# uzh-rpg/rpg_monocular_pose_estimator

Hardware: AMD Instinct MI355X
Metric: frames/sec at 752x480, 5 LEDs, brute-force init; pose RMSE vs CPU ref (higher is better)
Workload: dtype f64; 1 GPU; C2: 752x480 synthetic frames, 5 LEDs, 0 distractors, brute-force P3P init every frame, demo.launch parameters; frames_resident_in_hbm=True, side_streams_concurrent=1, scan_split_pct=28, side_scan_blocks=1, entry=mpe_estimate_batch_device_submit / _collect, parallelism=frames sharded over 1 GPU(s), pose records gathered to rank 0

## Files before the change

rpg_monocular_pose_estimator_amd/binding.py:

```python
import ctypes as C
import os
import re
import subprocess

import numpy as np

_HERE = os.path.dirname(os.path.abspath(__file__))
_CSRC = os.path.join(_HERE, "csrc")
_LIB = os.environ.get("MPE_LIB") or os.path.join(_HERE, "libmpe_hip.so")
_HEADER = os.path.join(os.path.dirname(_HERE), "include", "mpe.h")

MAX_MARKERS = 16
MAX_DETECTIONS = int(os.environ.get("MPE_MAX_DET", "64"))
WIDE_DETECTIONS = 256


class MpeError(RuntimeError):
    pass


class MpeParams(C.Structure):
    _fields_ = [
        ("threshold_value", C.c_int),
        ("gaussian_sigma", C.c_double),
        ("min_blob_area", C.c_double),
        ("max_blob_area", C.c_double),
        ("max_width_height_distortion", C.c_double),
        ("max_circular_distortion", C.c_double),
        ("back_projection_pixel_tolerance", C.c_double),
        ("nearest_neighbour_pixel_tolerance", C.c_double),
        ("certainty_threshold", C.c_double),
        ("valid_correspondence_threshold", C.c_double),
        ("roi_border_thickness", C.c_uint),
        ("histogram_threshold", C.c_uint),
    ]


class MpeResult(C.Structure):
    _fields_ = [("T", C.c_double * 16), ("cov", C.c_double * 36), ("status", C.c_int), ("n_det", C.c_int),
                ("n_corr", C.c_int), ("gn_iterations", C.c_int)]


class MpeDetections(C.Structure):
    _fields_ = [("n", C.c_int), ("status", C.c_int), ("undist_xy", C.c_double * (2 * MAX_DETECTIONS)),
                ("dist_xy", C.c_float * (2 * MAX_DETECTIONS))]


class MpeDetectionsWide(C.Structure):
    _fields_ = [("n", C.c_int), ("status", C.c_int), ("undist_xy", C.c_double * (2 * WIDE_DETECTIONS)),
                ("dist_xy", C.c_float * (2 * WIDE_DETECTIONS))]


RESULT_DTYPE = np.dtype([("T", "f8", (16,)), ("cov", "f8", (36,)), ("status", "i4"), ("n_det", "i4"),
                         ("n_corr", "i4"), ("gn_iterations", "i4")])
DETECTIONS_DTYPE = np.dtype([("n", "i4"), ("status", "i4"), ("undist_xy", "f8", (2 * MAX_DETECTIONS,)),
                             ("dist_xy", "f4", (2 * MAX_DETECTIONS,))])
assert RESULT_DTYPE.itemsize == C.sizeof(MpeResult)
DETECTIONS_WIDE_DTYPE = np.dtype([("n", "i4"), ("status", "i4"), ("undist_xy", "f8", (2 * WIDE_DETECTIONS,)),
                                  ("dist_xy", "f4", (2 * WIDE_DETECTIONS,))])
assert DETECTIONS_DTYPE.itemsize == C.sizeof(MpeDetections)
assert DETECTIONS_WIDE_DTYPE.itemsize == C.sizeof(MpeDetectionsWide)


def library_path():
    return _LIB


def build_library(force=False):
    cmd = ["make", "-s", "-j4", "-C", _CSRC] + (["-B"] if force else [])
    subprocess.check_call(cmd)
    if not os.path.exists(_LIB):
        raise MpeError("build did not produce %s" % _LIB)
    return _LIB


DEVICE_SOURCES = ("mpe_kernels_common.h", "mpe_k1.hip", "mpe_k2_head.h", "mpe_k2.hip", "mpe_k3.hip")


def device_source():
    out = []
    for name in DEVICE_SOURCES:
        with open(os.path.join(_CSRC, name)) as fh:
            txt = fh.read()
        txt = re.sub(r"//@file-prologue\n.*?//@file-prologue-end\n", "", txt, flags=re.S)
        txt = re.sub(r"//@file-epilogue\n.*?//@file-epilogue-end\n", "", txt, flags=re.S)
        if "//@include-k1b-dev" in txt:
            with open(os.path.join(_CSRC, "mpe_k1b_dev.h")) as fh:
                hdr = fh.read()
            body = hdr[hdr.index("//@k1b-dev-begin\n") + len("//@k1b-dev-begin\n"):hdr.index("//@k1b-dev-end\n")]
            txt = re.sub(r"//@include-k1b-dev.*?//@include-k1b-dev-end\n", lambda m: body, txt, count=1, flags=re.S)
        out.append(txt)
    return "".join(out)


def source_fingerprint():
    import hashlib
    hsh = hashlib.sha256()
    for name in DEVICE_SOURCES + ("mpe_k1b_dev.h", "mpe_ddmath.h", "mpe_p3p.h", "mpe_internal.h", "mpe_host.h", "mpe_schedule.cpp",
                                  "mpe_options.cpp", "mpe_track_abi.cpp", "mpe_abi.cpp", "mpe_track_device.hip",
                                  "mpe_gather.h", "mpe_pixel.h", "mpe_brute_blocks.h", "mpe_wide_peel.h", "mpe_wide.cpp"):
        with open(os.path.join(_CSRC, name), "rb") as fh:
            hsh.update(fh.read())
    return hsh.hexdigest()[:16]


def exported_symbols():
    txt = open(_HEADER).read()
    txt = re.sub(r"/\*.*?\*/", "", txt, flags=re.S)
    return sorted(set(re.findall(r"\b(mpe_[a-z0-9_]+)\s*\(", txt)))


_lib = None


def load_library():
    global _lib
    if _lib is not None:
        return _lib
    if not os.path.exists(_LIB):
        raise MpeError("%s is missing: run __graft_entry__.build() / make -C %s (there is no CPU fallback)"
                       % (_LIB, _CSRC))
    try:
        import torch
    except Exception:
        pass
    lib = C.CDLL(_LIB)
    lib.mpe_version.restype = C.c_char_p
    lib.mpe_last_error.restype = C.c_char_p
    lib.mpe_last_error.argtypes = [C.c_void_p]
    lib.mpe_get_stream.restype = C.c_void_p
    lib.mpe_get_stream.argtypes = [C.c_void_p]
    lib.mpe_create.argtypes = [C.POINTER(C.c_void_p), C.c_int]
    lib.mpe_destroy.argtypes = [C.c_void_p]
    lib.mpe_destroy.restype = None
    lib.mpe_set_stream.argtypes = [C.c_void_p, C.c_void_p]
    lib.mpe_synchronize.argtypes = [C.c_void_p]
    lib.mpe_set_profiling.argtypes = [C.c_void_p, C.c_int]
    lib.mpe_last_kernel_ms.argtypes = [C.c_void_p, C.POINTER(C.c_float)]
    lib.mpe_last_launch_shape.argtypes = [C.c_void_p, C.POINTER(C.c_int), C.POINTER(C.c_int)]
    lib.mpe_set_option.argtypes = [C.c_void_p, C.c_char_p, C.c_int]
    lib.mpe_default_params.argtypes = [C.POINTER(MpeParams)]
    lib.mpe_default_params.restype = None
    dp = C.POINTER(C.c_double)
    lib.mpe_find_leds.argtypes = [C.c_void_p, C.c_void_p, C.c_int, C.c_int, C.c_size_t, C.c_int, C.c_int, C.c_int,
                                  C.c_int, C.POINTER(MpeParams), dp, dp, C.c_int, dp, C.POINTER(C.c_float), C.c_int,
                                  C.POINTER(C.c_int)]
    lib.mpe_solve_bruteforce.argtypes = [C.c_void_p, dp, C.c_int, dp, C.c_int, dp, C.POINTER(MpeParams),
                                         C.POINTER(MpeResult), C.POINTER(C.c_uint32), C.POINTER(C.c_uint32)]
    ip, up = C.POINTER(C.c_int), C.POINTER(C.c_uint32)
    lib.mpe_solve_bruteforce_batch.argtypes = [C.c_void_p, dp, ip, C.c_int, dp, C.c_int, dp, C.POINTER(MpeParams),
                                               C.c_void_p, up, up]
    lib.mpe_solve_bruteforce_batch_setups.argtypes = [C.c_void_p, dp, ip, ip, C.c_int, C.c_void_p, C.c_int, C.c_void_p,
                                                      up, up]
    lib.mpe_estimate_batch.argtypes = [C.c_void_p, C.c_void_p, C.c_int, C.c_int, C.c_int, C.c_size_t, C.c_size_t,
                                       C.c_int, dp, C.c_int, dp, dp, C.c_int, C.POINTER(MpeParams), C.c_void_p]
    lib.mpe_estimate_batch_device.argtypes = [C.c_void_p, C.c_void_p, C.c_int, C.c_int, C.c_int, dp, C.c_int, dp, dp,
                                              C.c_int, C.POINTER(MpeParams), C.c_void_p]
    lib.mpe_estimate_batch_device_submit.argtypes = [C.c_void_p, C.c_void_p, C.c_int, C.c_int, C.c_int, dp, C.c_int, dp,
                                                     dp, C.c_int, C.POINTER(MpeParams), C.c_void_p, C.c_void_p, C.c_int]
    lib.mpe_estimate_batch_device_collect.argtypes = [C.c_void_p, C.c_void_p]
    lib.mpe_stream_next_ready.argtypes = [C.c_void_p, C.c_void_p]
    lib.mpe_stream_drop_prefetch.argtypes = [C.c_void_p]
    lib.mpe_track_step_batch_collect.argtypes = [C.c_void_p, C.c_void_p, C.c_void_p, C.c_void_p]
    lib.mpe_track_step_batch_cancel.argtypes = [C.c_void_p]
    lib.mpe_estimate_batch_multi_device_gather.argtypes = [C.c_void_p, C.c_int, C.c_void_p, C.c_void_p, C.c_int, C.c_int, dp,
                                                           C.c_int, dp, dp, C.c_int, C.POINTER(MpeParams), C.c_void_p,
                                                           C.POINTER(C.c_int)]
    lib.mpe_convert_to_mono8.argtypes = [C.c_void_p, C.c_void_p, C.c_int, C.c_int, C.c_int, C.c_int, C.c_int, C.c_int,
                                         C.c_size_t, C.c_size_t, C.c_void_p, C.c_int]
    lib.mpe_detect_batch.argtypes = [C.c_void_p, C.c_void_p, C.c_int, C.c_int, C.c_int, C.c_size_t, C.c_size_t, C.c_int,
                                     dp, dp, C.c_int, C.POINTER(MpeParams), C.c_void_p]
    lib.mpe_vote_batch.argtypes = [C.c_void_p, dp, C.POINTER(C.c_int), C.c_int, dp, C.c_int, dp, C.c_double,
                                   C.POINTER(C.c_uint32)]
    lib.mpe_vote_batch_wide.argtypes = lib.mpe_vote_batch.argtypes
    lib.mpe_detect_batch_wide.argtypes = lib.mpe_detect_batch.argtypes
    lib.mpe_estimate_batch_wide.argtypes = lib.mpe_estimate_batch.argtypes
    lib.mpe_solve_bruteforce_batch_wide.argtypes = lib.mpe_solve_bruteforce_batch.argtypes
    lib.mpe_vote_items.argtypes = [C.c_void_p, dp, C.POINTER(C.c_int), C.c_int, dp, C.c_int, dp, C.c_double,
                                   C.POINTER(C.c_int), C.POINTER(C.c_int), C.POINTER(C.c_uint32)]
    lib.mpe_check_and_refine.argtypes = [C.c_void_p, dp, C.c_int, dp, C.c_int, dp, C.POINTER(MpeParams),
                                         C.POINTER(C.c_uint32), C.c_int, C.POINTER(MpeResult)]
    lib.mpe_tracker_create.argtypes = [C.c_void_p, C.POINTER(C.c_void_p)]
    lib.mpe_tracker_destroy.argtypes = [C.c_void_p]
# ... 830 lines not shown
```

rpg_monocular_pose_estimator_amd/csrc/mpe_internal.h:

```cpp
#pragma once
#include <hip/hip_runtime.h>
#include <stdint.h>

#include "../../include/mpe.h"
#include "mpe_brute_blocks.h"

namespace mpe {

struct FrameGeom {
  int rows, cols, pitch;
  int segs_per_row;
  int segs_per_frame;
  int wb;
  int rw;
  int tw;
  int slot_cap;
};

struct DetectParams {
  int thr;
  int ksize;
  int taps[MPE_MAX_KSIZE];
  double min_area, max_area, max_wh, max_circ;
  double K[9];
  double ifx, ify;
  double k[8];
  int undist_iters;
  int roi_x, roi_y;
  unsigned taps_packed[2];
  int taps_u8;
};
inline void pack_taps(DetectParams& dp) {
  dp.taps_packed[0] = dp.taps_packed[1] = 0;
  dp.taps_u8 = 1;
  for (int i = 0; i < dp.ksize && i < MPE_MAX_KSIZE; ++i) {
    if (dp.taps[i] < 0 || dp.taps[i] > 255) dp.taps_u8 = 0;
    if (i < 8) dp.taps_packed[i >> 2] |= ((unsigned)dp.taps[i] & 0xFFu) << (8 * (i & 3));
  }
}

struct SolveParams {
  int n_markers;
  double markers[MPE_MAX_MARKERS * 3];
  double fx, fy, cx, cy;
  double back_tol;
  double certainty_thr;
  double valid_corr_thr;
  unsigned hist_thr;
  int vote_arith;
  int refine_variant;
};

__host__ __device__ inline bool vote_arith_is_strict(int a) { return a == 0 || a == 4; }
__host__ __device__ inline bool vote_arith_screens(int a) { return a == 1 || a == 3; }
__host__ __device__ inline bool vote_arith_glibc_pow(int a) { return a == 3 || a == 4; }

#define MPE_HIST_WORDS (MPE_MAX_DETECTIONS * MPE_MAX_MARKERS)
#define MPE_HIST_STRIDE (MPE_HIST_WORDS + 32)
#define MPE_WIDE_HIST_WORDS (MPE_WIDE_DETECTIONS * MPE_MAX_MARKERS)
#define MPE_WIDE_HIST_STRIDE (MPE_WIDE_HIST_WORDS + 32)

#define MPE_FIX_CTL_WORDS 8
struct VoteFixup {
  unsigned* ctl;
  unsigned long long* list;
  unsigned cap;
  unsigned screen;
};

int device_cu_count();
size_t k1b_scratch_bytes(const FrameGeom& g, int n_frames);
void k1b_set_general_blocks(int cap);
int k1b_get_general_blocks();
hipError_t launch_k1a_scan(const uint8_t* frames, size_t n_bytes, unsigned long long* flags, int thr,
                           int dummy_lds_bytes, hipStream_t s, int blocks_per_cu = 0);
hipError_t launch_k1b_blobs(const uint8_t* frames, const unsigned long long* flags, int n_frames, const FrameGeom& g,
                            const DetectParams& dp, mpe_detections* dets, int* worklist, uint8_t* scratch,
                            size_t scratch_bytes, int blob_hint, hipStream_t s, const void* frame_windows = nullptr,
                            bool lists_zeroed = false, bool first_tier_only = false, bool general_lds = false);
size_t k2_table_bytes(int n_markers);
hipError_t launch_k2_prep(const SolveParams& sp, double* tab, hipStream_t s);
hipError_t launch_k2_vote(mpe_detections* dets, int n_frames, const SolveParams& sp, const double* tab,
                          uint32_t* hist, int splits, int n_det_hint, hipStream_t s, const uint8_t* scan_px = nullptr,
                          size_t scan_bytes = 0, unsigned long long* scan_flags = nullptr, int scan_thr = 0,
                          size_t* scanned_bytes = nullptr, const int* item_range = nullptr,
                          const VoteFixup* fixup = nullptr);
hipError_t launch_k2_fixup(mpe_detections* dets, int n_frames, const SolveParams& sp, uint32_t* hist,
                           const VoteFixup& fixup, hipStream_t s, int relost_blocks = 32,
                           const int* item_range = nullptr);
int k2_table_slices(int n_markers);
size_t k3_mid_bytes(int n_frames);
hipError_t launch_k3_tail(const mpe_detections* dets, const uint32_t* hist, int n_frames, const SolveParams& sp,
                          mpe_result* results, uint32_t* corr_out, const uint32_t* corr_in, const double* nn_pred,
                          double nn_tol, void* mid_buf, hipStream_t s, int mode = 0);
struct TrackFramesArgs {
  const uint8_t* pix;
  size_t slot_bytes;
  const double* pred;
  const void* wins;
// ... 46 lines not shown
```

rpg_monocular_pose_estimator_amd/csrc/mpe_k1b_dev.h:

```cpp
#pragma once
#include "mpe_kernels_common.h"
namespace mpe {
struct BlobRec {
  long long a00, a10, a01;
  int xmin, xmax, ymin, ymax;
};
#ifndef K1B_ON_BLOBREC
#define K1B_ON_BLOBREC(rec, key)
#endif

__device__ __forceinline__ int reflect101(int p, int len) {
  if ((unsigned)p < (unsigned)len) return p;
  if (len == 1) return 0;
  do {
    p = (p < 0) ? -p : 2 * (len - 1) - p;
  } while ((unsigned)p >= (unsigned)len);
  return p;
}

__device__ __forceinline__ void lds_set_range(u64* bits, int lo, int hi) {
  const int wl = lo >> 6, wh = hi >> 6;
  if (wl == wh) {
    const u64 m = (~0ull << (lo & 63)) & (~0ull >> (63 - (hi & 63)));
    atomicOr(&bits[wl], m);
// ... 905 lines not shown
    if (over) st = MPE_FRAME_TOO_MANY_ROWS;
    out->status = st;
  }
}

struct FrameWin {
  int rows, cols, roi_x, roi_y;
};
__device__ __forceinline__ FrameGeom window_geom(const FrameGeom& g, const FrameWin* wins, int f, const DetectParams& dp,
                                                 int& roi_x, int& roi_y) {
  FrameGeom gl = g;
  roi_x = dp.roi_x;
  roi_y = dp.roi_y;
  if (wins) {
    const FrameWin w = wins[f];
    gl.rows = w.rows;
    gl.cols = w.cols;
    roi_x = w.roi_x;
    roi_y = w.roi_y;
  }
  return gl;
}

struct Island {
  short ylo, yhi;
  short clo, chi;
  short cfirst, clast;
  int pix_off, bm_off;
  int stage_end, blur_end;
  short blo, bhi;
};

#ifdef K1B_WIDE_WINDOWS
__device__ __forceinline__ int isl_xw0(const Island& is, int) { return 16 * is.clo; }
__device__ __forceinline__ int isl_words(const Island& is, int cols, int) {
  return ((min(cols - 1, 16 * is.chi + 15) - 16 * is.clo + 1) + 2 + 63) / 64;
}
#else
__device__ __forceinline__ int isl_xw0(const Island& is, int r) { return max(16 * is.clo, 16 * is.cfirst - r); }
__device__ __forceinline__ int isl_words(const Island& is, int cols, int r) {
  const int xhi = min(min(cols - 1, 16 * is.chi + 15), 16 * is.clast + 15 + r);
  return ((xhi - isl_xw0(is, r) + 1) + 2 + 63) / 64;
}
#endif
#ifndef K1B_SMALL_WAVES
#define K1B_SMALL_WAVES 1
#endif
#ifndef K1B_SMALL_MIN_WAVES
#define K1B_SMALL_MIN_WAVES 4
#endif
#ifndef K1B_SMALL_PIX
#define K1B_SMALL_PIX 4096
#endif
#ifndef K1B_SMALL_BM
#define K1B_SMALL_BM 208
#endif
struct K1bSmall {
  enum { PIX = K1B_SMALL_PIX, BM = K1B_SMALL_BM, SEG = 64, BAND = 8, ISL = 8, KEPT = 16, WAVES = K1B_SMALL_WAVES, MIN_WAVES = K1B_SMALL_MIN_WAVES };
};
struct K1bLarge {
  enum { PIX = 12288, BM = 704, SEG = 512, BAND = 32, ISL = 32, KEPT = 64, WAVES = 1, MIN_WAVES = 2 };
};


template <class C>
struct K1bWaveLds {
  enum { SCRATCH = 4 * C::SEG + 512 + 32 * C::BAND + 4 * C::BAND, POOL = C::PIX > SCRATCH ? C::PIX : SCRATCH };
  __attribute__((aligned(16))) uint8_t pool[POOL];
  int taps[MPE_MAX_KSIZE];
  int nseg, nband;
  int blur_go;
#ifdef K1B_PHASE_CLOCKS
  unsigned long long clk[8];
#endif
};
#ifdef K1B_PHASE_CLOCKS
#define K1B_PHASE_STAMP(W, i) \
  if ((threadIdx.x & 63) == 0) (W).clk[i] = __builtin_amdgcn_s_memtime();
#else
#define K1B_PHASE_STAMP(W, i)
#endif
template <class C>
struct K1bFrameLds {
  u64 nz[C::BM + 1], pm[C::BM + 1], ng[C::BM + 1];
  Island isl[C::ISL];
  float kx[C::KEPT], ky[C::KEPT];
  unsigned kkey[C::KEPT];
  int nkept, over, nisl;
  int ready, cols, roi_x, roi_y;
};

#ifdef K1B_STOP_AFTER
#define K1B_STOP_POINT(PHASE, REC) \
  if (K1B_STOP_AFTER <= (PHASE)) { \
    if (lane == 0) {               \
      (REC)->n = 0;                \
      (REC)->status = 0;           \
    }                              \
    return false;                  \
  }
#else
#define K1B_STOP_POINT(PHASE, REC)
#endif
template <class C>
__device__ __forceinline__ void k1b_blur_items(K1bWaveLds<C>& W, K1bFrameLds<C>& S, const FrameGeom& g, const DetectParams& dp,
                                               int tid, int nthr) {
  const Island* s_isl = S.isl;
  const int nisl = S.nisl, r = dp.ksize / 2;
  const int tot_blur = s_isl[nisl - 1].blur_end;
  for (int i = tid; i < tot_blur; i += nthr) {
    int k = 0;
    while (i >= s_isl[k].blur_end) ++k;
    const Island is = s_isl[k];
    const int li = i - (k ? s_isl[k - 1].blur_end : 0);
    const int ncols = is.bhi - is.blo + 1;
    const int yb = li / ncols, c = is.blo + (li - yb * ncols);
    const int H = is.yhi - is.ylo + 1;
    const int Wd = isl_words(is, g.cols, r);
    const PixWin pw = {W.pool + is.pix_off, is.ylo, H, is.cfirst, 16 * (is.clast - is.cfirst + 1), 0u, nullptr, 0};
    blur_to_bitmap(pw, g.rows, g.cols, dp, W.taps, is.ylo + yb, c, S.nz + is.bm_off + (size_t)(yb + 1) * Wd, isl_xw0(is, r));
  }
}

template <class C, bool HELP = false>
__device__ __forceinline__ bool k1b_front(const int f, const uint8_t* __restrict__ frames, size_t slot_bytes,
                                          const u64* __restrict__ flags, const FrameGeom& g, const DetectParams& dp,
                                          mpe_detections* __restrict__ dets, int* __restrict__ worklist,
                                          K1bWaveLds<C>& W, K1bFrameLds<C>& S) {
  const int lane = threadIdx.x & 63;
  unsigned* s_seg = reinterpret_cast<unsigned*>(W.pool);
  u64* s_rowact = reinterpret_cast<u64*>(W.pool + 4 * C::SEG);
  u64(*s_colocc)[4] = reinterpret_cast<u64(*)[4]>(W.pool + 4 * C::SEG + 512);
  short* s_bandlo = reinterpret_cast<short*>(W.pool + 4 * C::SEG + 512 + 32 * C::BAND);
  short* s_bandhi = s_bandlo + C::BAND;
  uint8_t* s_pix = W.pool;
  int& s_nseg = W.nseg;
  int& s_nband = W.nband;
  u64 *s_nz = S.nz, *s_pm = S.pm, *s_ng = S.ng;
  Island* s_isl = S.isl;
  int& s_nkept = S.nkept;
  int& s_over = S.over;
  int& s_nisl = S.nisl;
  const uint8_t* frame = frames + (size_t)f * slot_bytes;
  mpe_detections* out = dets + f;
  const int r = dp.ksize / 2;
  const int dc = (r + 15) / 16;
  const int spr = g.segs_per_row;
  const unsigned add = (unsigned)(255 - dp.thr) * 0x00010001u;

  s_rowact[lane] = 0;
  for (int i = lane; i < C::BAND * 4; i += 64) (&s_colocc[0][0])[i] = 0;
  if (lane == 0) {
    s_nseg = 0;
    s_nkept = 0;
    s_over = 0;
    s_nband = 0;
    s_nisl = 0;
  }
  wave_sync();

  {
    const size_t G0 = (size_t)f * g.segs_per_frame;
    const int nwin = (g.segs_per_frame + 63) >> 6;
    const size_t w0 = G0 >> 6;
    const int sh = (int)(G0 & 63);
    for (int i0 = 0; i0 < nwin; i0 += 256) {
      u64 v[4];
#pragma unroll
      for (int k = 0; k < 4; ++k) {
        const int i = i0 + 64 * k + lane;
        v[k] = 0;
        if (i < nwin) {
          const u64 a = flags[w0 + i], b = flags[w0 + i + 1];
          v[k] = sh ? ((a >> sh) | (b << (64 - sh))) : a;
          const int rem = g.segs_per_frame - i * 64;
          if (rem < 64) v[k] &= (1ull << rem) - 1;
        }
      }
#pragma unroll
      for (int k = 0; k < 4; ++k) {
        u64 vv = v[k];
        const int i = i0 + 64 * k + lane;
        while (vv) {
          const int s = i * 64 + __builtin_ctzll(vv);
          vv &= vv - 1;
          const int y0 = s / spr, c0 = s - y0 * spr;
          const int slot = atomicAdd(&s_nseg, 1);
          if (slot < C::SEG) s_seg[slot] = ((unsigned)y0 << 16) | (unsigned)c0;
          lds_set_range(s_rowact, max(0, y0 - r), min(g.rows - 1, y0 + r));
        }
      }
    }
  }
  wave_sync();
  const int nseg = s_nseg;
  if (nseg == 0) {
    if (lane == 0) {
      out->n = 0;
      out->status = 0;
    }
    return false;
  }
  K1B_STOP_POINT(1, out)
  K1B_PHASE_STAMP(W, 1)
  bool fallback = nseg > C::SEG;
  int why = fallback ? 1 : 0;

  {
    const u64 act = (lane < g.rw) ? s_rowact[lane] : 0;
    const u64 prevw = (lane > 0 && lane < g.rw) ? s_rowact[lane - 1] : 0;
    const u64 nextw = (lane + 1 < g.rw) ? s_rowact[lane + 1] : 0;
    u64 st = act & ~((act << 1) | (prevw >> 63));
    u64 en = act & ~((act >> 1) | (nextw << 63));
    const int cs = __builtin_popcountll(st), ce = __builtin_popcountll(en);
    int ps = cs, pe = ce;
#pragma unroll
    for (int d = 1; d < 64; d <<= 1) {
      const int a = __shfl_up(ps, d), b = __shfl_up(pe, d);
      if (lane >= d) {
        ps += a;
        pe += b;
      }
    }
    int is_ = ps - cs, ie = pe - ce;
    if (!fallback) {
      while (st) {
        const int b = __builtin_ctzll(st);
        st &= st - 1;
        if (is_ < C::BAND) s_bandlo[is_] = (short)(lane * 64 + b);
        ++is_;
      }
      while (en) {
        const int b = __builtin_ctzll(en);
        en &= en - 1;
        if (ie < C::BAND) s_bandhi[ie] = (short)(lane * 64 + b);
        ++ie;
      }
    }
    if (lane == 63) s_nband = ps;
  }
  wave_sync();
  const int nband = s_nband;
  fallback = fallback || nband > C::BAND;
  if (fallback && !why) why = 2;

  if (!fallback) {
    for (int i = lane; i < nseg; i += 64) {
      const unsigned sg = s_seg[i];
      const int y = (int)(sg >> 16), c = (int)(sg & 0xFFFF);
      int b = 0;
      while (b < nband - 1 && y > s_bandhi[b]) ++b;
      atomicOr(&s_colocc[b][c >> 6], 1ull << (c & 63));
    }
  }
  wave_sync();

  if (!fallback && lane < nband) {
    const int ylo = s_bandlo[lane], yhi = s_bandhi[lane];
    for (int cstart = 0; cstart < spr;) {
      int cfirst = -1;
      for (int wi = cstart >> 6; wi < 4 && wi * 64 < spr; ++wi) {
        u64 w = s_colocc[lane][wi];
        if (wi == (cstart >> 6)) w &= ~0ull << (cstart & 63);
        if (w) {
          cfirst = wi * 64 + __builtin_ctzll(w);
          break;
        }
      }
      if (cfirst < 0) break;
      int clast = cfirst;
      for (;;) {
        int nxt = -1;
        for (int c = clast + 1; c <= min(spr - 1, clast + 2 * dc + 1); ++c)
          if ((s_colocc[lane][c >> 6] >> (c & 63)) & 1) {
            nxt = c;
            break;
          }
        if (nxt < 0) break;
        clast = nxt;
      }
      cstart = clast + 2 * dc + 2;
      const int idx = atomicAdd(&s_nisl, 1);
      if (idx < C::ISL) {
        Island is;
        is.ylo = (short)ylo;
        is.yhi = (short)yhi;
        is.cfirst = (short)cfirst;
        is.clast = (short)clast;
        is.clo = (short)max(0, cfirst - dc);
        is.chi = (short)min(spr - 1, clast + dc);
        is.pix_off = is.bm_off = is.stage_end = is.blur_end = 0;
        is.blo = is.clo;
        is.bhi = is.chi;
        s_isl[idx] = is;
      }
    }
  }
  wave_sync();
  const int nisl = s_nisl;
  fallback = fallback || nisl > C::ISL;
  if (fallback && !why) why = 3;

  if (!fallback) {
    int pixb = 0, bmw = 0, nst = 0, nbl = 0;
    if (lane < nisl) {
      const Island is = s_isl[lane];
      const int H = is.yhi - is.ylo + 1;
      const int W = isl_words(is, g.cols, r);
      const int nbs = is.clast - is.cfirst + 1;
      pixb = H * 16 * nbs;
      bmw = (H + 2) * W;
      nst = H * nbs;
      nbl = H * (is.chi - is.clo + 1);
    }
    int ip = pixb, ib = bmw, is_ = nst, il = nbl;
#pragma unroll
    for (int d = 1; d < 32; d <<= 1) {
      const int a = __shfl_up(ip, d), b = __shfl_up(ib, d), c = __shfl_up(is_, d), e = __shfl_up(il, d);
      if (lane >= d) {
        ip += a;
        ib += b;
        is_ += c;
        il += e;
      }
    }
    if (lane < nisl) {
      s_isl[lane].pix_off = ip - pixb;
      s_isl[lane].bm_off = ib - bmw;
      s_isl[lane].stage_end = is_;
      s_isl[lane].blur_end = il;
    }
    const int tot_pix = __shfl(ip, nisl - 1), tot_bm = __shfl(ib, nisl - 1);
    fallback = tot_pix > C::PIX || tot_bm > C::BM;
    if (fallback) why = tot_pix > C::PIX ? 4 : 5;
  }
  if (fallback) {
    if (lane == 0) {
      out->n = 0;
      out->status = MPE_FRAME_TOO_MANY_ROWS;
      if (worklist) {
        const int k = atomicAdd(&worklist[0], 1);
        worklist[1 + k] = f | (why << 24);
      }
    }
    return false;
  }
  wave_sync();
  K1B_STOP_POINT(2, out)
  K1B_PHASE_STAMP(W, 2)

  {
    const int tot_bm = s_isl[nisl - 1].bm_off +
                       (s_isl[nisl - 1].yhi - s_isl[nisl - 1].ylo + 3) * isl_words(s_isl[nisl - 1], g.cols, r);
    for (int i = lane; i < tot_bm; i += 64) {
      s_nz[i] = 0;
      s_pm[i] = 0;
      s_ng[i] = 0;
    }
    const int tot_stage = s_isl[nisl - 1].stage_end;
    for (int i = lane; i < tot_stage; i += 64) {
      int k = 0;
      while (i >= s_isl[k].stage_end) ++k;
      const Island is = s_isl[k];
      const int li = i - (k ? s_isl[k - 1].stage_end : 0);
      const int nbs = is.clast - is.cfirst + 1;
      const int yb = li / nbs, sc = li - yb * nbs;
      uint4 v = *reinterpret_cast<const uint4*>(frame + (size_t)(is.ylo + yb) * g.pitch + 16 * (is.cfirst + sc));
      v.x = tozero4(v.x, add);
      v.y = tozero4(v.y, add);
      v.z = tozero4(v.z, add);
      v.w = tozero4(v.w, add);
      *reinterpret_cast<uint4*>(s_pix + is.pix_off + (size_t)yb * 16 * nbs + 16 * sc) = v;
    }
  }
  wave_sync();
  K1B_STOP_POINT(3, out)
  K1B_PHASE_STAMP(W, 3)

#ifdef K1B_BLUR_NARROWING
  if (dc == 1) {
    int nbl = 0;
    if (lane < nisl) {
      Island is = s_isl[lane];
      const int H = is.yhi - is.ylo + 1, nbs = is.clast - is.cfirst + 1;
      const bool may_l = is.clo < is.cfirst && 16 * (is.cfirst - 1) >= r;
      const bool may_r = is.chi > is.clast && 16 * (is.clast + 2) + r <= g.cols;
      if (may_l || may_r) {
        unsigned left = 0, right = 0;
        const uint8_t* base = s_pix + is.pix_off;
        for (int yb = 0; yb < H; ++yb) {
          const uint8_t* rowp = base + (size_t)yb * 16 * nbs;
          for (int k = 0; k < r; ++k) {
            left |= rowp[k];
            right |= rowp[16 * nbs - 1 - k];
          }
        }
        if (may_l && !left) is.blo = is.cfirst;
        if (may_r && !right) is.bhi = is.clast;
        s_isl[lane].blo = is.blo;
        s_isl[lane].bhi = is.bhi;
      }
      nbl = H * (is.bhi - is.blo + 1);
    }
    int il = nbl;
#pragma unroll
    for (int d = 1; d < 32; d <<= 1) {
      const int e = __shfl_up(il, d);
      if (lane >= d) il += e;
    }
    if (lane < nisl) s_isl[lane].blur_end = il;
    wave_sync();
  }
#endif

  if constexpr (HELP) {
    if (lane == 0) W.blur_go = 1;
    __syncthreads();
    k1b_blur_items<C>(W, S, g, dp, (int)threadIdx.x, (int)blockDim.x);
    __syncthreads();
  } else {
    k1b_blur_items<C>(W, S, g, dp, lane, 64);
  }
  wave_sync();
  K1B_STOP_POINT(4, out)
  K1B_PHASE_STAMP(W, 4)
  return true;
}

__device__ __forceinline__ void k1b_hand_over(int f, mpe_detections* __restrict__ dets, int* __restrict__ worklist) {
  dets[f].n = 0;
  dets[f].status = MPE_FRAME_TOO_MANY_ROWS;
  if (worklist) {
    const int k = atomicAdd(&worklist[0], 1);
    worklist[1 + k] = f | (6 << 24);
  }
}

template <class C, bool HELP = false>
__device__ __forceinline__ void k1b_wave(const int f, const bool valid, const uint8_t* __restrict__ frames,
                                         const u64* __restrict__ flags, const FrameGeom& gslot, const DetectParams& dp,
                                         mpe_detections* __restrict__ dets, int* __restrict__ worklist,
                                         const FrameWin* __restrict__ wins) {
  __shared__ K1bWaveLds<C> Wl[C::WAVES];
  __shared__ K1bFrameLds<C> Sl[C::WAVES];
  static_assert(!HELP || C::WAVES == 1, "helper waves: one frame per block");
  const int lane = threadIdx.x & 63;
  const int wv = C::WAVES > 1 ? __builtin_amdgcn_readfirstlane((int)(threadIdx.x >> 6)) : 0;
  K1bWaveLds<C>& W = Wl[wv];
  K1bFrameLds<C>& S = Sl[wv];
// ... 110 lines not shown
```

rpg_monocular_pose_estimator_amd/csrc/mpe_schedule.cpp:

```cpp
#include "mpe_host.h"

namespace mpe_host {

int fail(mpe_handle* h, int code, const char* what, hipError_t e) {
  if (h) {
    h->err = what;
    if (e != hipSuccess) {
      h->err += ": ";
      h->err += hipGetErrorString(e);
    }
  }
  return code;
}


int enter(mpe_handle* h) {
  hipError_t e = hipSetDevice(h->device);
  if (e != hipSuccess) return fail(h, MPE_ERR_HIP, "hipSetDevice", e);
  if (h->tail_sub_pending) {
    e = hipStreamWaitEvent(h->stream, h->tail_sub_done[h->tail_last], 0);
    if (e != hipSuccess) return fail(h, MPE_ERR_HIP, "hipStreamWaitEvent", e);
    h->tail_sub_pending = false;
  }
  return MPE_OK;
// ... 8 lines not shown
  const hipError_t e = hipHostMalloc(&h->mailbox, want, hipHostMallocDefault);
  if (e != hipSuccess) return fail(h, MPE_ERR_HIP, "hipHostMalloc (staging memory)", e);
  h->mailbox_cap = want;
  return MPE_OK;
}

unsigned factorial_u32(int n) {
  unsigned r = 1;
  for (int i = 2; i <= n; ++i) r *= (unsigned)i;
  return r;
}
unsigned num_combinations_u32(unsigned n, unsigned k) {
  const unsigned den = factorial_u32((int)k) * factorial_u32((int)(n - k));
  return den ? factorial_u32((int)n) / den : 0u;
}

int gaussian_taps(double sigma, int* taps) {
  if (!(sigma > 0)) return -1;
  const int n = (int)std::lrint(sigma * 3 * 2 + 1) | 1;
  if (n > MPE_MAX_KSIZE) return -1;
  float cf[MPE_MAX_KSIZE];
  const double scale2x = -0.5 / (sigma * sigma);
  double sum = 0;
  for (int i = 0; i < n; ++i) {
    const double x = i - (n - 1) * 0.5;
    cf[i] = (float)std::exp(scale2x * x * x);
    sum += cf[i];
  }
  sum = 1. / sum;
  for (int i = 0; i < n; ++i) {
    cf[i] = (float)(cf[i] * sum);
    taps[i] = (int)std::lrint((double)cf[i] * 256.0);
  }
  return n;
}

int make_detect_params(const mpe_params* p, const double K[9], const double* D, int nD, int roi_x, int roi_y,
                       DetectParams& dp) {
  std::memset(&dp, 0, sizeof(dp));
  dp.thr = p->threshold_value < -1 ? -1 : (p->threshold_value > 255 ? 255 : p->threshold_value);
  dp.ksize = gaussian_taps(p->gaussian_sigma, dp.taps);
  if (dp.ksize < 0) return -1;
  pack_taps(dp);
  dp.min_area = p->min_blob_area;
  dp.max_area = p->max_blob_area;
  dp.max_wh = p->max_width_height_distortion;
  dp.max_circ = p->max_circular_distortion;
  for (int i = 0; i < 9; ++i) dp.K[i] = K[i];
  dp.ifx = 1. / K[0];
  dp.ify = 1. / K[4];
  for (int i = 0; i < 8; ++i) dp.k[i] = (D && i < nD) ? D[i] : 0.0;
  dp.undist_iters = (D && nD > 0) ? 5 : 0;
  dp.roi_x = roi_x;
  dp.roi_y = roi_y;
  return 0;
}

int make_solve_params(const mpe_handle* h, const mpe_params* p, const double* markers, int n_markers, const double K[9],
                      SolveParams& sp) {
  if (n_markers < 0 || n_markers > MPE_MAX_MARKERS) return -1;
  std::memset(&sp, 0, sizeof(sp));
  sp.n_markers = n_markers;
  for (int i = 0; i < 3 * n_markers; ++i) sp.markers[i] = markers[i];
  sp.fx = K[0];
  sp.fy = K[4];
  sp.cx = K[2];
  sp.cy = K[5];
  sp.back_tol = p->back_projection_pixel_tolerance;
  sp.certainty_thr = p->certainty_threshold;
  sp.valid_corr_thr = p->valid_correspondence_threshold;
  sp.hist_thr = p->histogram_threshold ? p->histogram_threshold : num_combinations_u32((unsigned)n_markers, 3);
  sp.vote_arith = h->vote_arith;
  sp.refine_variant = h->refine_variant;
  return 0;
}

int make_geom(const mpe_handle* h, int rows, int cols, FrameGeom& g) {
  if (rows <= 0 || cols <= 0 || rows > 4096 || cols > 4000) return -1;
  g.rows = rows;
  g.cols = cols;
  g.pitch = (cols + 15) & ~15;
  g.segs_per_row = g.pitch / 16;
  g.segs_per_frame = rows * g.segs_per_row;
  g.wb = (cols + 2 + 63) / 64 + 1;
  g.rw = (rows + 63) / 64;
  g.tw = (g.segs_per_row + 63) / 64;
  const size_t per_slot = (size_t)(3 * g.wb + g.tw) * 8 + (size_t)g.wb / 8 + 1;
  size_t fixed = 2 * (size_t)g.rw * 8 + 2 * (size_t)g.rw * 4 + 64;
  long cap = ((long)h->lds_budget - (long)fixed) / (long)per_slot;
  if (cap > rows + 2 + rows / 2) cap = rows + 2 + rows / 2;
  if (cap < 8) return -1;
  g.slot_cap = (int)cap;
  return 0;
}

size_t flag_words(size_t n_bytes) {
  const size_t n_seg = n_bytes / 16;
  return ((n_seg + 511) / 512) * 8 + 8;
}

int stage_frames(mpe_handle* h, const uint8_t* frames, int n_frames, int rows, int cols, size_t stride,
                 size_t frame_stride, int on_device, int roi_x, int roi_y, int roi_w, int roi_h, const FrameGeom& g,
                 const uint8_t** d_out) {
  const bool full = (roi_x == 0 && roi_y == 0 && roi_w == cols && roi_h == rows);
  const bool packed = full && stride == (size_t)g.pitch && frame_stride == (size_t)rows * g.pitch &&
                      (reinterpret_cast<uintptr_t>(frames) & 15) == 0 && g.pitch == cols;
  if (on_device && packed) {
    *d_out = frames;
    return MPE_OK;
  }
  const size_t bytes = (size_t)n_frames * g.rows * g.pitch;
  HIP_TRY(h, h->frames.reserve(bytes + 16));
  uint8_t* dst = static_cast<uint8_t*>(h->frames.p);
  if (on_device) {
    HIP_TRY(h, launch_repack(frames, stride, frame_stride, n_frames, roi_x, roi_y, roi_w, roi_h, dst, g.pitch,
                             h->stream));
  } else {
    if (g.pitch != roi_w) HIP_TRY(h, hipMemsetAsync(dst, 0, bytes, h->stream));
    if (full && stride == (size_t)cols && frame_stride == (size_t)rows * cols && g.pitch == cols) {
      HIP_TRY(h, hipMemcpyAsync(dst, frames, bytes, hipMemcpyHostToDevice, h->stream));
    } else {
      for (int f = 0; f < n_frames; ++f) {
        const uint8_t* src = frames + (size_t)f * frame_stride + (size_t)roi_y * stride + roi_x;
        HIP_TRY(h, hipMemcpy2DAsync(dst + (size_t)f * g.rows * g.pitch, g.pitch, src, stride, roi_w, roi_h,
                                    hipMemcpyHostToDevice, h->stream));
      }
    }
  }
  *d_out = dst;
  return MPE_OK;
}

bool general_lds_now(const mpe_handle* h) {
  if (h->general_lds >= 0) return h->general_lds != 0;
  return h->gen_seen_host && *h->gen_seen_host > 0;
}
hipError_t general_seen_copy(mpe_handle* h, const int* worklist, int n_frames, hipStream_t st) {
  if (!h->gen_seen_host) {
    const hipError_t e = hipHostMalloc(reinterpret_cast<void**>(&h->gen_seen_host), 64, hipHostMallocDefault);
    if (e != hipSuccess) return e;
    *h->gen_seen_host = 0;
  }
  return hipMemcpyAsync(h->gen_seen_host, worklist + (n_frames + 1), sizeof(int), hipMemcpyDeviceToHost, st);
}

int det_hint_for(const mpe_handle* h, int n_markers) {
  const int v = h->detections_hint > 0 ? h->detections_hint : h->det_seen;
  return std::min(MPE_FAST_VOTE_DETECTIONS, std::max(n_markers, v));
}

int auto_splits(const mpe_handle* h, int n_frames, int n_markers) {
  if (h->vote_splits > 0) return h->vote_splits;
  if (!vote_arith_is_strict(h->vote_arith) && h->vote_splits == 0) {
    const int slices = k2_table_slices(n_markers);
    if (slices > 0) return -slices;
  }
  if (n_frames >= 1024 || n_markers <= 5) return 1;
  int s = 2048 / std::max(1, n_frames);
  return std::max(1, std::min(s, 64));
}

int fix_counter_sum(mpe_handle* h, int which, unsigned long long& out) {
  out = which == 1 ? h->fix_overflow_base : which == 6 ? h->fix_relost_base : which == 7 ? h->fix_wide_base : h->fix_items_base;
  if (!h->fix.p) return MPE_OK;
  HIP_TRY(h, hipDeviceSynchronize());
  unsigned ctl[mpe_handle::kMaxSub * MPE_FIX_CTL_WORDS];
// ... 664 lines not shown
```

Baseline: 14.61 million frames/s.

## Streamline k1b segment extraction with wave scans, magic division and vector zeroing

```diff
diff --git a/rpg_monocular_pose_estimator_amd/binding.py b/rpg_monocular_pose_estimator_amd/binding.py
--- a/rpg_monocular_pose_estimator_amd/binding.py
+++ b/rpg_monocular_pose_estimator_amd/binding.py
@@ -98,7 +98,8 @@
     hsh = hashlib.sha256()
     for name in DEVICE_SOURCES + ("mpe_k1b_dev.h", "mpe_ddmath.h", "mpe_p3p.h", "mpe_internal.h", "mpe_host.h", "mpe_schedule.cpp",
                                   "mpe_options.cpp", "mpe_track_abi.cpp", "mpe_abi.cpp", "mpe_track_device.hip",
-                                  "mpe_gather.h", "mpe_pixel.h", "mpe_brute_blocks.h", "mpe_wide_peel.h", "mpe_wide.cpp"):
+                                  "mpe_gather.h", "mpe_pixel.h", "mpe_brute_blocks.h", "mpe_wide_peel.h", "mpe_wide.cpp",
+                                  "mpe_seg_div.h"):
         with open(os.path.join(_CSRC, name), "rb") as fh:
             hsh.update(fh.read())
     return hsh.hexdigest()[:16]
diff --git a/rpg_monocular_pose_estimator_amd/csrc/mpe_internal.h b/rpg_monocular_pose_estimator_amd/csrc/mpe_internal.h
--- a/rpg_monocular_pose_estimator_amd/csrc/mpe_internal.h
+++ b/rpg_monocular_pose_estimator_amd/csrc/mpe_internal.h
@@ -4,6 +4,7 @@
 
 #include "../../include/mpe.h"
 #include "mpe_brute_blocks.h"
+#include "mpe_seg_div.h"
 
 namespace mpe {
 
@@ -15,6 +16,8 @@
   int rw;
   int tw;
   int slot_cap;
+  unsigned spr_mul;
+  int spr_shift;
 };
 
 struct DetectParams {
diff --git a/rpg_monocular_pose_estimator_amd/csrc/mpe_k1b_dev.h b/rpg_monocular_pose_estimator_amd/csrc/mpe_k1b_dev.h
--- a/rpg_monocular_pose_estimator_amd/csrc/mpe_k1b_dev.h
+++ b/rpg_monocular_pose_estimator_amd/csrc/mpe_k1b_dev.h
@@ -1011,7 +1011,9 @@
 #endif
 template <class C>
 struct K1bFrameLds {
-  u64 nz[C::BM + 1], pm[C::BM + 1], ng[C::BM + 1];
+  enum { BMW = (C::BM + 2) & ~1 };
+  __attribute__((aligned(16))) u64 nz[BMW];
+  u64 pm[BMW], ng[BMW];
   Island isl[C::ISL];
   float kx[C::KEPT], ky[C::KEPT];
   unsigned kkey[C::KEPT];
@@ -1063,7 +1065,6 @@
   short* s_bandlo = reinterpret_cast<short*>(W.pool + 4 * C::SEG + 512 + 32 * C::BAND);
   short* s_bandhi = s_bandlo + C::BAND;
   uint8_t* s_pix = W.pool;
-  int& s_nseg = W.nseg;
   int& s_nband = W.nband;
   u64 *s_nz = S.nz, *s_pm = S.pm, *s_ng = S.ng;
   Island* s_isl = S.isl;
@@ -1080,7 +1081,6 @@
   s_rowact[lane] = 0;
   for (int i = lane; i < C::BAND * 4; i += 64) (&s_colocc[0][0])[i] = 0;
   if (lane == 0) {
-    s_nseg = 0;
     s_nkept = 0;
     s_over = 0;
     s_nband = 0;
@@ -1088,24 +1088,60 @@
   }
   wave_sync();
 
+  int nseg = 0;
   {
     const size_t G0 = (size_t)f * g.segs_per_frame;
     const int nwin = (g.segs_per_frame + 63) >> 6;
-    const size_t w0 = G0 >> 6;
+    const u64* __restrict__ fw = flags + (G0 >> 6);
     const int sh = (int)(G0 & 63);
+    const int nload = nwin + (sh ? 1 : 0);
+    const unsigned dmul = g.spr_mul;
+    const int dsh = g.spr_shift;
     for (int i0 = 0; i0 < nwin; i0 += 256) {
       u64 v[4];
 #pragma unroll
       for (int k = 0; k < 4; ++k) {
         const int i = i0 + 64 * k + lane;
-        v[k] = 0;
-        if (i < nwin) {
-          const u64 a = flags[w0 + i], b = flags[w0 + i + 1];
-          v[k] = sh ? ((a >> sh) | (b << (64 - sh))) : a;
-          const int rem = g.segs_per_frame - i * 64;
-          if (rem < 64) v[k] &= (1ull << rem) - 1;
+        v[k] = i < nload ? fw[i] : 0;
+      }
+      if (sh) {
+        const u64 nxt = i0 + 256 < nload ? fw[i0 + 256] : 0;
+#pragma unroll
+        for (int k = 0; k < 4; ++k) {
+          u64 up0 = nxt;
+          if (k < 3)
+            up0 = (u64)__builtin_amdgcn_readfirstlane((unsigned)v[k < 3 ? k + 1 : k]) |
+                  ((u64)__builtin_amdgcn_readfirstlane((unsigned)(v[k < 3 ? k + 1 : k] >> 32)) << 32);
+          unsigned blo = __shfl_down((unsigned)v[k], 1);
+          unsigned bhi = sh > 32 ? __shfl_down((unsigned)(v[k] >> 32), 1) : 0u;
+          if (lane == 63) {
+            blo = (unsigned)up0;
+            bhi = (unsigned)(up0 >> 32);
+          }
+          v[k] = (v[k] >> sh) | ((((u64)bhi << 32) | blo) << (64 - sh));
         }
       }
+      int cnt = 0;
+#pragma unroll
+      for (int k = 0; k < 4; ++k) {
+        const int i = i0 + 64 * k + lane;
+        const int rem = g.segs_per_frame - i * 64;
+        if (rem <= 0)
+          v[k] = 0;
+        else if (rem < 64)
+          v[k] &= (1ull << rem) - 1;
+        cnt += __builtin_popcountll(v[k]);
+      }
+      if (__builtin_amdgcn_ballot_w64(cnt != 0) == 0) continue;
+      int inc = cnt;
+#pragma unroll
+      for (int d = 1; d < 64; d <<= 1) {
+        const int a = __shfl_up(inc, d);
+        if (lane >= d) inc += a;
+      }
+      int slot = nseg + inc - cnt;
+      nseg += __builtin_amdgcn_readlane(inc, 63);
+      int ymark = -1;
 #pragma unroll
       for (int k = 0; k < 4; ++k) {
         u64 vv = v[k];
@@ -1113,16 +1149,18 @@
         while (vv) {
           const int s = i * 64 + __builtin_ctzll(vv);
           vv &= vv - 1;
-          const int y0 = s / spr, c0 = s - y0 * spr;
-          const int slot = atomicAdd(&s_nseg, 1);
+          const int y0 = seg_row(s, dmul, dsh), c0 = s - y0 * spr;
           if (slot < C::SEG) s_seg[slot] = ((unsigned)y0 << 16) | (unsigned)c0;
-          lds_set_range(s_rowact, max(0, y0 - r), min(g.rows - 1, y0 + r));
+          ++slot;
+          if (y0 != ymark) {
+            lds_set_range(s_rowact, max(0, y0 - r), min(g.rows - 1, y0 + r));
+            ymark = y0;
+          }
         }
       }
     }
   }
   wave_sync();
-  const int nseg = s_nseg;
   if (nseg == 0) {
     if (lane == 0) {
       out->n = 0;
@@ -1142,15 +1180,13 @@
     u64 st = act & ~((act << 1) | (prevw >> 63));
     u64 en = act & ~((act >> 1) | (nextw << 63));
     const int cs = __builtin_popcountll(st), ce = __builtin_popcountll(en);
-    int ps = cs, pe = ce;
+    int pse = cs | (ce << 16);
 #pragma unroll
     for (int d = 1; d < 64; d <<= 1) {
-      const int a = __shfl_up(ps, d), b = __shfl_up(pe, d);
-      if (lane >= d) {
-        ps += a;
-        pe += b;
-      }
-    }
+      const int a = __shfl_up(pse, d);
+      if (lane >= d) pse += a;
+    }
+    const int ps = pse & 0xFFFF, pe = pse >> 16;
     int is_ = ps - cs, ie = pe - ce;
     if (!fallback) {
       while (st) {
@@ -1174,38 +1210,49 @@
   if (fallback && !why) why = 2;
 
   if (!fallback) {
-    for (int i = lane; i < nseg; i += 64) {
-      const unsigned sg = s_seg[i];
+    const int bhi_l = lane < nband ? (int)s_bandhi[lane] : 0x7fffffff;
+    for (int i0 = 0; i0 < nseg; i0 += 64) {
+      const int i = i0 + lane;
+      const unsigned sg = i < nseg ? s_seg[i] : 0u;
       const int y = (int)(sg >> 16), c = (int)(sg & 0xFFFF);
       int b = 0;
-      while (b < nband - 1 && y > s_bandhi[b]) ++b;
-      atomicOr(&s_colocc[b][c >> 6], 1ull << (c & 63));
+      for (int j = 0; j < nband - 1; ++j) b += (y > __builtin_amdgcn_readlane(bhi_l, j)) ? 1 : 0;
+      if (i < nseg) atomicOr(&s_colocc[b][c >> 6], 1ull << (c & 63));
     }
   }
   wave_sync();
 
   if (!fallback && lane < nband) {
     const int ylo = s_bandlo[lane], yhi = s_bandhi[lane];
+    const int nocc = (spr + 63) >> 6;
+    const u64 occ0 = s_colocc[lane][0];
+    u64 occ1 = 0, occ2 = 0, occ3 = 0;
+    if (nocc > 1) {
+      occ1 = s_colocc[lane][1];
+      occ2 = s_colocc[lane][2];
+      occ3 = s_colocc[lane][3];
+    }
+    auto next_occupied = [&](int from) -> int {
+      int res = -1;
+      if (nocc > 1) {
+        const u64 w3 = from >= 256 ? 0 : from > 192 ? occ3 & (~0ull << (from - 192)) : occ3;
+        if (w3) res = 192 + __builtin_ctzll(w3);
+        const u64 w2 = from >= 192 ? 0 : from > 128 ? occ2 & (~0ull << (from - 128)) : occ2;
+        if (w2) res = 128 + __builtin_ctzll(w2);
+        const u64 w1 = from >= 128 ? 0 : from > 64 ? occ1 & (~0ull << (from - 64)) : occ1;
+        if (w1) res = 64 + __builtin_ctzll(w1);
+      }
+      const u64 w0 = from >= 64 ? 0 : occ0 & (~0ull << from);
+      if (w0) res = __builtin_ctzll(w0);
+      return res;
+    };
     for (int cstart = 0; cstart < spr;) {
-      int cfirst = -1;
-      for (int wi = cstart >> 6; wi < 4 && wi * 64 < spr; ++wi) {
-        u64 w = s_colocc[lane][wi];
-        if (wi == (cstart >> 6)) w &= ~0ull << (cstart & 63);
-        if (w) {
-          cfirst = wi * 64 + __builtin_ctzll(w);
-          break;
-        }
-      }
+      const int cfirst = next_occupied(cstart);
       if (cfirst < 0) break;
       int clast = cfirst;
       for (;;) {
-        int nxt = -1;
-        for (int c = clast + 1; c <= min(spr - 1, clast + 2 * dc + 1); ++c)
-          if ((s_colocc[lane][c >> 6] >> (c & 63)) & 1) {
-            nxt = c;
-            break;
-          }
-        if (nxt < 0) break;
+        const int nxt = next_occupied(clast + 1);
+        if (nxt < 0 || nxt > clast + 2 * dc + 1) break;
         clast = nxt;
       }
       cstart = clast + 2 * dc + 2;
@@ -1230,6 +1277,7 @@
   fallback = fallback || nisl > C::ISL;
   if (fallback && !why) why = 3;
 
+  int stage_end_l = 0;
   if (!fallback) {
     int pixb = 0, bmw = 0, nst = 0, nbl = 0;
     if (lane < nisl) {
@@ -1244,7 +1292,7 @@
     }
     int ip = pixb, ib = bmw, is_ = nst, il = nbl;
 #pragma unroll
-    for (int d = 1; d < 32; d <<= 1) {
+    for (int d = 1; d < C::ISL; d <<= 1) {
       const int a = __shfl_up(ip, d), b = __shfl_up(ib, d), c = __shfl_up(is_, d), e = __shfl_up(il, d);
       if (lane >= d) {
         ip += a;
@@ -1259,6 +1307,7 @@
       s_isl[lane].stage_end = is_;
       s_isl[lane].blur_end = il;
     }
+    stage_end_l = is_;
     const int tot_pix = __shfl(ip, nisl - 1), tot_bm = __shfl(ib, nisl - 1);
     fallback = tot_pix > C::PIX || tot_bm > C::BM;
     if (fallback) why = tot_pix > C::PIX ? 4 : 5;
@@ -1281,19 +1330,33 @@
   {
     const int tot_bm = s_isl[nisl - 1].bm_off +
                        (s_isl[nisl - 1].yhi - s_isl[nisl - 1].ylo + 3) * isl_words(s_isl[nisl - 1], g.cols, r);
-    for (int i = lane; i < tot_bm; i += 64) {
-      s_nz[i] = 0;
-      s_pm[i] = 0;
-      s_ng[i] = 0;
-    }
-    const int tot_stage = s_isl[nisl - 1].stage_end;
+    {
+      const uint4 z = make_uint4(0u, 0u, 0u, 0u);
+      uint4 *znz = reinterpret_cast<uint4*>(s_nz), *zpm = reinterpret_cast<uint4*>(s_pm), *zng = reinterpret_cast<uint4*>(s_ng);
+      for (int i = lane; 2 * i < tot_bm; i += 64) {
+        znz[i] = z;
+        zpm[i] = z;
+        zng[i] = z;
+      }
+    }
+    const int tot_stage = __builtin_amdgcn_readlane(stage_end_l, nisl - 1);
     for (int i = lane; i < tot_stage; i += 64) {
-      int k = 0;
-      while (i >= s_isl[k].stage_end) ++k;
+      int k = 0, first = 0;
+      for (int j = 0; j < nisl - 1; ++j) {
+        const int e = __builtin_amdgcn_readlane(stage_end_l, j);
+        if (i >= e) {
+          ++k;
+          first = e;
+        }
+      }
       const Island is = s_isl[k];
-      const int li = i - (k ? s_isl[k - 1].stage_end : 0);
+      const int li = i - first;
       const int nbs = is.clast - is.cfirst + 1;
-      const int yb = li / nbs, sc = li - yb * nbs;
+      int yb = li, sc = 0;
+      if (nbs != 1) {
+        yb = li / nbs;
+        sc = li - yb * nbs;
+      }
       uint4 v = *reinterpret_cast<const uint4*>(frame + (size_t)(is.ylo + yb) * g.pitch + 16 * (is.cfirst + sc));
       v.x = tozero4(v.x, add);
       v.y = tozero4(v.y, add);
diff --git a/rpg_monocular_pose_estimator_amd/csrc/mpe_schedule.cpp b/rpg_monocular_pose_estimator_amd/csrc/mpe_schedule.cpp
--- a/rpg_monocular_pose_estimator_amd/csrc/mpe_schedule.cpp
+++ b/rpg_monocular_pose_estimator_amd/csrc/mpe_schedule.cpp
@@ -114,6 +114,8 @@
   g.pitch = (cols + 15) & ~15;
   g.segs_per_row = g.pitch / 16;
   g.segs_per_frame = rows * g.segs_per_row;
+  seg_div_magic(g.segs_per_row, g.spr_mul, g.spr_shift);
+  if ((unsigned long long)g.segs_per_frame > seg_div_exact_below(g.segs_per_row, g.spr_mul, g.spr_shift)) return -1;
   g.wb = (cols + 2 + 63) / 64 + 1;
   g.rw = (rows + 63) / 64;
   g.tw = (g.segs_per_row + 63) / 64;
diff --git a/rpg_monocular_pose_estimator_amd/csrc/mpe_seg_div.h b/rpg_monocular_pose_estimator_amd/csrc/mpe_seg_div.h
--- /dev/null
+++ b/rpg_monocular_pose_estimator_amd/csrc/mpe_seg_div.h
@@ -0,0 +1,25 @@
+#pragma once
+#ifdef __HIPCC__
+#define MPE_SEG_DIV_FN __host__ __device__ __forceinline__
+#else
+#define MPE_SEG_DIV_FN inline
+#endif
+namespace mpe {
+
+inline void seg_div_magic(int d, unsigned& mul, int& shift) {
+  int l = 0;
+  while ((1 << l) < d) ++l;
+  shift = 31 + l;
+  mul = (unsigned)((((unsigned long long)1 << shift) + (unsigned long long)d - 1) / (unsigned long long)d);
+}
+inline unsigned long long seg_div_exact_below(int d, unsigned mul, int shift) {
+  const unsigned long long e = (unsigned long long)mul * (unsigned long long)d - ((unsigned long long)1 << shift);
+  if (e == 0) return (unsigned long long)1 << 32;
+  const unsigned long long lim = (((unsigned long long)1 << shift) + e - 1) / e;
+  return lim < ((unsigned long long)1 << 32) ? lim : (unsigned long long)1 << 32;
+}
+MPE_SEG_DIV_FN int seg_row(int s, unsigned mul, int shift) {
+  return (int)(((unsigned long long)(unsigned)s * mul) >> shift);
+}
+
+}
```

Result: no change. 14.57 million frames/s (-0.2%).
